# adamjorr/kbbq

Hardware: AMD Instinct MI355X
Metric: recalibrated Gbases/sec (higher is better)
Workload: dtype u64

## Files before the change

### kbbq_amd/csrc/bucket.h

```cpp
#pragma once
#include <hip/hip_runtime.h>
#include <stdint.h>

#include "device_common.h"

namespace kbbq {

constexpr int SUB_BITS = 12;
constexpr int NB2_BITS = 9;
constexpr int SUB_BLOCKS = 1 << SUB_BITS;
constexpr int NB2 = 1 << NB2_BITS;
constexpr int L1_SHIFT = SUB_BITS + NB2_BITS;
constexpr int MAX_NB1 = 512;
constexpr int N_XCD = 8;
constexpr int CNT_STRIDE = 32;
constexpr int BK_THREADS = 512;
constexpr int EMIT_GRID = 512;

struct BucketDev {
    unsigned long long *l1;
    uint32_t *l1_cnt;
    uint32_t *l2;
    uint32_t *l2_cnt;
    uint32_t *tickets;
    unsigned long long *direct;
    uint32_t cap1, cap2;
    int nb1;
    int n_src;
    int cnt_stride;
    uint32_t n_sub;
};

__device__ __forceinline__ int xcc_id() {
    unsigned x;
    asm volatile("s_getreg_b32 %0, hwreg(HW_REG_XCC_ID, 0, 4)" : "=s"(x));
    return (int)(x & (N_XCD - 1));
}

__device__ __forceinline__ uint32_t block_scan512(uint32_t v, uint32_t *wave_tot, uint32_t *total) {
    const int lane = threadIdx.x & 63, w = threadIdx.x >> 6;
    uint32_t inc = v;
#pragma unroll
    for (int o = 1; o < 64; o <<= 1) { const uint32_t y = __shfl_up(inc, o); if (lane >= o) inc += y; }
    if (lane == 63) wave_tot[w] = inc;
    __syncthreads();
    uint32_t before = 0, all = 0;
#pragma unroll
    for (int i = 0; i < 8; ++i) { const uint32_t t = wave_tot[i]; before += i < w ? t : 0; all += t; }
    *total = all;
    return before + inc - v;
}

template <int NW, int CH, bool BY_BASE, int RPW, bool PRIV, bool DENSE = true>
__global__ void __launch_bounds__(BK_THREADS) k_emit_marked(ReadsDev R, KParams K, FiltDev F, BucketDev B, const uint64_t *mask,
                                                             uint64_t mask_words, const uint64_t *kofs,
                                                             unsigned long long *inserted) {
    using S = Stage<NW>;
    constexpr int SLOTS = RPW * CH;
    extern __shared__ unsigned long long sorted[];
    __shared__ uint32_t stage[8][DENSE ? RPW : 1][2 * S::WORDS];
    __shared__ uint32_t hist[MAX_NB1], ofs_l[MAX_NB1], gbase_l[MAX_NB1], fill_l[MAX_NB1], wave_tot[8];
    const int lane = threadIdx.x & 63;
    const int w = __builtin_amdgcn_readfirstlane(threadIdx.x >> 6);
    uint32_t *L32 = stage[w][0];
    const int k = K.k;
    const int src = PRIV ? (int)blockIdx.x : xcc_id();
    const uint64_t reads_per_tile = 8 * RPW;
    const uint64_t n_tiles = (R.n_reads + reads_per_tile - 1) / reads_per_tile;
    unsigned long long mine = 0, direct = 0;
    hist[threadIdx.x] = 0;
    if (PRIV) fill_l[threadIdx.x] = (int)threadIdx.x < B.nb1 ? B.l1_cnt[(size_t)src * B.nb1 + threadIdx.x] : 0u;
    __syncthreads();
    uint64_t off[RPW], kb[RPW], word[RPW];
    uint32_t len[RPW];
    auto fetch_tile = [&](uint64_t tile) {
        const uint64_t r0 = (tile * 8 + w) * RPW;
#pragma unroll
        for (int rr = 0; rr < RPW; ++rr) {
            off[rr] = 0; kb[rr] = 0; word[rr] = 0; len[rr] = 0;
            if (r0 + rr < R.n_reads) {
                read_span(R, r0 + rr, off[rr], len[rr]);
                kb[rr] = BY_BASE ? off[rr] : kmer_base(kofs, r0 + rr, R.read_len, k);
                word[rr] = stage_fetch<NW>(R, nullptr, mask, kb[rr], mask_words - 1, off[rr], lane);
            }
        }
    };
    if (blockIdx.x < n_tiles) fetch_tile(blockIdx.x);
    for (uint64_t tile = blockIdx.x; tile < n_tiles; tile += gridDim.x) {
        unsigned long long rec[SLOTS];
        int rk[SLOTS];
#pragma unroll
        for (int s = 0; s < SLOTS; ++s) { rec[s] = 0; rk[s] = -1; }
        if (DENSE) {
            unsigned long long *wlist = sorted + (size_t)w * SLOTS * 64;
            int n_dense = 0;
            __builtin_amdgcn_wave_barrier();
            if (lane < S::WORDS) {
#pragma unroll
                for (int rr = 0; rr < RPW; ++rr) stage_store(stage[w][rr], lane, word[rr]);
            }
            __builtin_amdgcn_wave_barrier();
#pragma unroll
            for (int rr = 0; rr < RPW; ++rr) {
                const int nk = (int)len[rr] - k + 1;
                if (nk > 0) {
                    const uint32_t *L32 = stage[w][rr];
                    const int o31 = (int)(off[rr] & 31), o63 = (int)(off[rr] & 63), x63 = (int)(kb[rr] & 63);
#pragma unroll
                    for (int c = 0; c < CH; ++c) {
                        if (c * 64 < nk) {
                            const int s = c * 64 + lane;
                            const bool marked = lds_bit(L32 + 2 * S::X, x63 + s) != 0;
                            const bool valid = (lds_window32(L32 + 2 * S::M, o63 + s) & K.nmask_bits) == 0;
                            const bool take = s < nk && marked && (BY_BASE || valid);
                            const unsigned long long bal = __ballot(take);
                            if (take) wlist[n_dense + __popcll(bal & ((1ULL << lane) - 1))] = lds_window64(L32 + 2 * S::B, 2 * (o31 + s));
                            n_dense += (int)__popcll(bal);
                            if (!BY_BASE && R.hint_sampled) or_bits64(R.hint_sampled, off[rr] + (uint64_t)c * 64, bal, lane);
                            mine += __popcll(bal);
                        }
                    }
                }
            }
            __builtin_amdgcn_wave_barrier();
#pragma unroll
            for (int i = 0; i < SLOTS; ++i) {
                if (i * 64 < n_dense && i * 64 + lane < n_dense) {
                    const uint64_t key = canon_key(wlist[i * 64 + lane], K);
                    const uint32_t blk = block_of(F, key);
                    rec[i] = ((unsigned long long)blk << 16) | pattern_of(F, key);
                    rk[i] = (int)atomicAdd(&hist[blk >> L1_SHIFT], 1u);
                }
            }
        } else {
#pragma unroll
        for (int rr = 0; rr < RPW; ++rr) {
            const int nk = (int)len[rr] - k + 1;
            if (nk > 0) {
                __builtin_amdgcn_wave_barrier();
                if (lane < S::WORDS) stage_store(L32, lane, word[rr]);
                __builtin_amdgcn_wave_barrier();
                const int o31 = (int)(off[rr] & 31), o63 = (int)(off[rr] & 63), x63 = (int)(kb[rr] & 63);
#pragma unroll
                for (int c = 0; c < CH; ++c) {
                    if (c * 64 < nk) {
                        const int s = c * 64 + lane;
                        const bool marked = lds_bit(L32 + 2 * S::X, x63 + s) != 0;
                        const bool valid = (lds_window32(L32 + 2 * S::M, o63 + s) & K.nmask_bits) == 0;
                        const bool take = s < nk && marked && (BY_BASE || valid);
                        const uint64_t key = canon_key(lds_window64(L32 + 2 * S::B, 2 * (o31 + s)), K);
                        const uint32_t blk = block_of(F, key);
                        rec[rr * CH + c] = ((unsigned long long)blk << 16) | pattern_of(F, key);
                        if (take) rk[rr * CH + c] = (int)atomicAdd(&hist[blk >> L1_SHIFT], 1u);
                        const unsigned long long bal = __ballot(take);
                        if (!BY_BASE && R.hint_sampled) or_bits64(R.hint_sampled, off[rr] + (uint64_t)c * 64, bal, lane);
                        mine += __popcll(bal);
                    }
                }
            }
        }
        }
        if (tile + gridDim.x < n_tiles) fetch_tile(tile + gridDim.x);
        __syncthreads();
        const uint32_t cnt = hist[threadIdx.x];
        hist[threadIdx.x] = 0;
        uint32_t g = 0;
        if (PRIV) {
            g = fill_l[threadIdx.x];
            fill_l[threadIdx.x] = g + cnt;
        } else if (cnt) {
            g = atomicAdd(&B.l1_cnt[((size_t)src * B.nb1 + threadIdx.x) * CNT_STRIDE], cnt);
        }
        uint32_t total;
        const uint32_t ex = block_scan512(cnt, wave_tot, &total);
        ofs_l[threadIdx.x] = ex;
        gbase_l[threadIdx.x] = g;
        __syncthreads();
#pragma unroll
        for (int s = 0; s < SLOTS; ++s)
            if (rk[s] >= 0) sorted[ofs_l[(uint32_t)(rec[s] >> (16 + L1_SHIFT))] + (uint32_t)rk[s]] = rec[s];
        __syncthreads();
        for (uint32_t i = threadIdx.x; i < total; i += BK_THREADS) {
            const unsigned long long v = sorted[i];
            const uint32_t b = (uint32_t)(v >> (16 + L1_SHIFT));
            const uint32_t pos = gbase_l[b] + (i - ofs_l[b]);
            if (pos < B.cap1) {
                B.l1[((size_t)src * B.nb1 + b) * B.cap1 + pos] = v;
            } else {
                bloom_put(F, (uint32_t)(v >> 16), (uint32_t)(v & 0xFFFFu));
                ++direct;
            }
        }
        if (DENSE) __syncthreads();
    }
    if (PRIV && (int)threadIdx.x < B.nb1) B.l1_cnt[(size_t)src * B.nb1 + threadIdx.x] = fill_l[threadIdx.x];
    if (inserted && lane == 0 && mine) atomicAdd(inserted, mine);
    if (direct) atomicAdd(B.direct, direct);
}

constexpr int SPLIT_PER_THREAD = 12;
constexpr int SPLIT_TILE = BK_THREADS * SPLIT_PER_THREAD;

__global__ void __launch_bounds__(BK_THREADS) k_split(FiltDev F, BucketDev B, uint32_t chunks_per_region) {
    __shared__ uint32_t hist[NB2], ofs_l[NB2], gbase_l[NB2], wave_tot[8], unit_l;
    __shared__ uint32_t sorted[SPLIT_TILE];
    __shared__ uint16_t sorted_b[SPLIT_TILE];
    const int home = xcc_id();
    unsigned long long direct = 0;
    hist[threadIdx.x] = 0;
    for (int qi = 0; qi < N_XCD; ++qi) {
        const int q = (home + qi) & (N_XCD - 1);
        const uint32_t n_buckets = B.nb1 > q ? (uint32_t)(B.nb1 - q + N_XCD - 1) / N_XCD : 0;
        const uint32_t n_units = n_buckets * (uint32_t)B.n_src * chunks_per_region;
        for (;;) {
            __syncthreads();
            if (threadIdx.x == 0) unit_l = atomicAdd(&B.tickets[q * CNT_STRIDE], 1u);
            __syncthreads();
            const uint32_t unit = unit_l;
            if (unit >= n_units) break;
            const uint32_t chunk = unit % chunks_per_region, rest = unit / chunks_per_region;
            const int x = (int)(rest % (uint32_t)B.n_src), b1 = q + (int)(rest / (uint32_t)B.n_src) * N_XCD;
            const size_t region = (size_t)x * B.nb1 + b1;
            const uint32_t n = min(B.l1_cnt[region * B.cnt_stride], B.cap1);
            const uint32_t first = chunk * (uint32_t)SPLIT_TILE;
            if (first >= n) continue;
            const uint32_t m = min((uint32_t)SPLIT_TILE, n - first);
            const unsigned long long *src = B.l1 + region * B.cap1 + first;
            uint32_t rec[SPLIT_PER_THREAD];
            int rk[SPLIT_PER_THREAD];
#pragma unroll
            for (int j = 0; j < SPLIT_PER_THREAD; ++j) {
                const uint32_t i = j * BK_THREADS + threadIdx.x;
// ... 92 lines not shown
```

### kbbq_amd/csrc/engine.hip

```cpp
#include <hip/hip_runtime.h>

#include <algorithm>
#include <cstdarg>
#include <cstdio>
#include <cstdlib>
#include <cstring>
#include <map>
#include <mutex>
#include <string>
#include <thread>
#include <vector>

#include "../../include/kbbq_engine.h"
#include "abi_internal.h"
#include "correct.h"
#include "correct_wave.h"
#include "device_common.h"
#include "host_model.h"

using namespace kbbq;

static thread_local char g_err[512] = "";
int kbbq_fail(int code, const char *fmt, ...) {
    va_list ap;
// ... 24 lines not shown
    uint64_t table_bytes() const { return spec.n_blocks * kEngineBlockBytes; }
    FiltDev dev() const {
        FiltDev f;
        f.table = reinterpret_cast<ulonglong2 *>(d_table);
        f.patterns = reinterpret_cast<const ulonglong2 *>(d_patterns);
        f.n_blocks = spec.n_blocks;
        const ModMagic mm = make_mod_magic(spec.n_blocks);
        f.mod_magic = mm.m64;
        f.mod_m32 = mm.m32;
        f.salt0 = spec.salt[0];
        f.salt1 = spec.salt[1];
        return f;
    }
};

struct ProfileSlot {
    std::string name;
    uint64_t launches = 0;
    double ms = 0;
};
struct PendingEvent {
    int slot;
    hipEvent_t a, b;
};

struct Options {
    bool no_overlap = false;
    bool no_fastpath = false;
    bool lane_walk = false;
    bool no_pass4_pipeline = false;
    int pass2_side = 2;
    bool tally_general = false;
    bool infer_subset = true;
    bool debug_bucket = false;
    int bucket = -1;
    uint64_t bucket_records = 0;
    uint64_t pass4_piece = 0;
    int scan_blocks = -1;
    int walk_blocks = -1;
    int infer_blocks = 0;
};

struct kbbq_engine {
    kbbq_params p;
    Options opt;
    KParams K;
    hipStream_t stream = nullptr;
    hipStream_t stream2 = nullptr;
    hipEvent_t ev_main = nullptr, ev_side[2] = {nullptr, nullptr};
    hipEvent_t ev_draw = nullptr, ev_ins[2] = {nullptr, nullptr};
    bool ins_pending[2] = {false, false};
    int draw_turn = 0;
    bool side_busy[2] = {false, false};
    bool pass3_shared = false;
    unsigned long long *d_totals = nullptr;
    int side_turn = 0;
    uint32_t *d_qpresent = nullptr;
    uint32_t qpresent[8] = {};
    bool qpresent_known = false;
    uint8_t *d_dq_qslot = nullptr;
    int dq_slots = 0;
    uint32_t *d_rg_present[2] = {nullptr, nullptr};
    hipStream_t cur = nullptr;
    unsigned long long *cur_cnt = nullptr;
    FilterHost filt[2];
    Xoshiro256 seed_state;
    uint64_t draw_threshold = 0;
    bool draw_always = false;
    bool thresholds_set = false;
    std::vector<int32_t> thresholds;
    unsigned long long *d_hist = nullptr;
    uint64_t hist_cycle_words = 0, hist_dinuc_words = 0;
    DqTables dq;
// ... 552 lines not shown

int kbbq_engine_create(const kbbq_params *params, kbbq_engine **out) {
    if (!params || !out) return fail(KBBQ_EINVAL, "null argument");
    if (params->k < 1 || params->k > KBBQ_MAX_KMER) return fail(KBBQ_ERANGE, "k must be <= %d and > 0", KBBQ_MAX_KMER);
    if (params->n_rg < 1 || params->n_rg > 65535) return fail(KBBQ_EINVAL, "n_rg must be in 1..65535");
    if (params->max_read_len < 1 || params->max_read_len > KBBQ_MAX_READ_LEN)
        return fail(KBBQ_ERANGE, "max_read_len must be in 1..%d", KBBQ_MAX_READ_LEN);
    int ndev = 0;
    if (hipGetDeviceCount(&ndev) != hipSuccess || ndev == 0) return fail(KBBQ_ENODEV, "no HIP device visible");
    if (params->device < 0 || params->device >= ndev) return fail(KBBQ_ENODEV, "device %d of %d", params->device, ndev);
    DeviceGuard create_guard(params->device);
    HIP_TRY(create_guard.err);
    kbbq_engine *e = new kbbq_engine;
    e->p = *params;
    {
        Options &o = e->opt;
        auto env_set = [](const char *name) { const char *v = getenv(name); return v && *v; };
        auto env_int = [](const char *name, int dflt) { const char *v = getenv(name); return v && *v ? atoi(v) : dflt; };
        const int fl = params->flags;
        o.no_overlap = (fl & KBBQ_F_NO_OVERLAP) || env_set("KBBQ_NO_OVERLAP");
        o.no_fastpath = (fl & KBBQ_F_NO_FASTPATH) || env_set("KBBQ_NO_FASTPATH");
        o.lane_walk = (fl & KBBQ_F_LANE_WALK) || (getenv("KBBQ_CORRECT") && !strcmp(getenv("KBBQ_CORRECT"), "lane"));
        o.no_pass4_pipeline = (fl & KBBQ_F_NO_PASS4_PIPELINE) || env_set("KBBQ_NO_PASS4_PIPELINE");
        o.pass2_side = (fl & KBBQ_F_PASS2_INORDER) ? 0 : env_int("KBBQ_PASS2_SIDE", o.pass2_side);
        o.tally_general = env_set("KBBQ_TALLY_GENERAL");
        o.infer_subset = env_int("KBBQ_INFER_SUBSET", 1) != 0;
        o.debug_bucket = env_set("KBBQ_DEBUG_BUCKET");
        o.bucket = (fl & KBBQ_F_BUCKET_ON) ? 1 : (fl & KBBQ_F_BUCKET_OFF) ? 0 : env_set("KBBQ_BUCKET") ? (env_int("KBBQ_BUCKET", 0) != 0 ? 1 : 0) : -1;
        o.bucket_records = env_u64("KBBQ_BUCKET_RECORDS", 0);
        o.pass4_piece = env_u64("KBBQ_PASS4_PIECE", 0);
        o.scan_blocks = env_int("KBBQ_SCAN_BLOCKS", o.scan_blocks);
        o.walk_blocks = env_int("KBBQ_WALK_BLOCKS", o.walk_blocks);
        o.infer_blocks = env_int("KBBQ_INFER_BLOCKS", o.infer_blocks);
    }
    e->K.k = params->k;
    e->K.shift = 2u * (unsigned)(params->k - 1);
    e->K.mask = params->k < 32 ? ((1ULL << (2 * params->k)) - 1) : ~0ULL;
    e->K.nmask_bits = params->k < 32 ? ((1u << params->k) - 1) : 0xFFFFFFFFu;
    const double fprs[2] = {params->fpr_sampled, params->fpr_trusted};
    for (int w = 0; w < 2; ++w) {
        if (!make_filter_spec(params->approx_kmers, fprs[w], params->bloom_seed, e->filt[w].spec)) {
            delete e;
            return fail(KBBQ_EINVAL, "Error: Invalid bloom filter parameters. Adjust parameters and try again.");
        }
    }
    hipError_t he = hipStreamCreateWithFlags(&e->stream, hipStreamNonBlocking);
    if (he == hipSuccess) he = hipStreamCreateWithFlags(&e->stream2, hipStreamNonBlocking);
    if (he == hipSuccess) he = hipEventCreateWithFlags(&e->ev_main, hipEventDisableTiming);
    if (he == hipSuccess) he = hipEventCreateWithFlags(&e->ev_draw, hipEventDisableTiming);
    for (int t = 0; t < 2 && he == hipSuccess; ++t) he = hipEventCreateWithFlags(&e->ev_ins[t], hipEventDisableTiming);
    if (he == hipSuccess) he = hipEventCreateWithFlags(&e->ev_side[0], hipEventDisableTiming);
    if (he == hipSuccess) he = hipEventCreateWithFlags(&e->ev_side[1], hipEventDisableTiming);
    if (he == hipSuccess) he = hipStreamCreateWithFlags(&e->copy, hipStreamNonBlocking);
    if (he == hipSuccess) he = hipEventCreateWithFlags(&e->bk.ev_flush, hipEventDisableTiming);
    if (he == hipSuccess) he = hipEventCreateWithFlags(&e->bk.ev_est, hipEventDisableTiming);
    if (he == hipSuccess) he = hipEventCreateWithFlags(&e->ev_infer, hipEventDisableTiming);
    for (int t = 0; t < 2 && he == hipSuccess; ++t) he = hipEventCreateWithFlags(&e->ev_take[t], hipEventDisableTiming);
    if (he == hipSuccess) he = hipHostMalloc((void **)&e->bk.h_inserted, 64, hipHostMallocDefault);
    for (int i = 0; i < 3 && he == hipSuccess; ++i) {
        he = hipEventCreateWithFlags(&e->slot[i].h2d, hipEventDisableTiming);
        if (he == hipSuccess) he = hipEventCreateWithFlags(&e->slot[i].d2h, hipEventDisableTiming);
        for (int t = 0; t < 2 && he == hipSuccess; ++t) he = hipEventCreateWithFlags(&e->slot[i].done[t], hipEventDisableTiming);
    }
    e->cur = e->stream;
    if (he != hipSuccess) { kbbq_engine_destroy(e); return fail(KBBQ_EIO, "hipStreamCreate: %s", hipGetErrorString(he)); }
#define CREATE_TRY(expr)                                                                           \
// ... 123 lines not shown
    e->dq_set = false;
    memset(e->stats, 0, sizeof e->stats);
    return sync_engine(e);
}

int kbbq_engine_sync(kbbq_engine *e) {
    ENGINE_DEVICE(e);
    { int frc = bucket_flush_all(e); if (frc) return frc; }
    if (!e) return fail(KBBQ_EINVAL, "null engine");
    return sync_engine(e);
}

void *kbbq_engine_stream(kbbq_engine *e) { return e ? (void *)e->stream : nullptr; }

int kbbq_engine_dims(kbbq_engine *e, uint64_t *n_rg, uint64_t *n_cycle) {
    if (!e) return fail(KBBQ_EINVAL, "null engine");
    if (n_rg) *n_rg = (uint64_t)e->p.n_rg;
    if (n_cycle) *n_cycle = (uint64_t)e->p.max_read_len;
    return KBBQ_OK;
}

int kbbq_engine_tune(kbbq_engine *e, const char *name, uint64_t value) {
    if (!e || !name) return fail(KBBQ_EINVAL, "null argument");
    if (!strcmp(name, "bucket_records")) {
        if (e->bk.allocated) return fail(KBBQ_ESTATE, "the record buffers are allocated already");
        e->opt.bucket_records = value;
    } else if (!strcmp(name, "pass4_piece")) {
        e->opt.pass4_piece = value;
    } else if (!strcmp(name, "scan_blocks") || !strcmp(name, "walk_blocks") || !strcmp(name, "infer_blocks")) {
        if (value > 17) return fail(KBBQ_EINVAL, "%s: 0 (as many as fit) to 16 workgroups per CU, 17 = default", name);
        (name[0] == 's' ? e->opt.scan_blocks : name[0] == 'w' ? e->opt.walk_blocks : e->opt.infer_blocks) = value == 17 ? (name[0] == 'i' ? 0 : -1) : (int)value;
    } else if (!strcmp(name, "infer_subset")) {
        e->opt.infer_subset = value != 0;
    } else if (!strcmp(name, "pass2_side")) {
        ENGINE_DEVICE(e);
        { int frc = bucket_flush_all(e); if (frc) return frc; }
        int rc = sync_engine(e);
        if (rc) return rc;
        if (value > 2) return fail(KBBQ_EINVAL, "pass2_side: 0, 1 or 2");
        e->opt.pass2_side = (int)value;
        e->bk.stream[0] = e->bk.stream[1] = nullptr;
    } else if (!strcmp(name, "no_overlap")) {
        ENGINE_DEVICE(e);
        { int frc = bucket_flush_all(e); if (frc) return frc; }
        int rc = sync_engine(e);
        if (rc) return rc;
        e->opt.no_overlap = value != 0;
        e->bk.stream[0] = e->bk.stream[1] = nullptr;
    } else {
        return fail(KBBQ_EINVAL, "unknown knob '%s'", name);
    }
    return KBBQ_OK;
}

int kbbq_filter_info_get(kbbq_engine *e, int which, kbbq_filter_info *out) {
    ENGINE_DEVICE(e);
    { int frc = bucket_flush_all(e); if (frc) return frc; }
    if (!e || !out || which < 0 || which > 1) return fail(KBBQ_EINVAL, "bad argument");
    const FilterSpec &s = e->filt[which].spec;
    memset(out, 0, sizeof *out);
    out->bits = s.bits;
    out->bits_unblocked = s.bits_unblocked;
    out->n_blocks = s.n_blocks;
    out->table_bytes = e->filt[which].table_bytes();
    out->random_seed = s.random_seed;
    out->n_hash = s.n_hash;
// ... 459 lines not shown

int kbbq_count_kmer_positions(kbbq_engine *e, const kbbq_reads *reads, uint64_t *out) {
    ENGINE_DEVICE(e);
    if (!e || !reads || !out) return fail(KBBQ_EINVAL, "null argument");
    HostBatchDone host_done(e, reads);
    ReadsDev R; int max_len;
    int rc = device_view(e, reads, &R, &max_len, false);
    if (rc) return rc;
    const uint64_t *kofs;
    return kmer_prefix(e, R, &kofs, out);
}

}

constexpr int kStagedMax = 512;
constexpr int kTallyMaxWindows = 24;
template <template <int> class Launcher, typename... Args>
static int dispatch_nw(int max_len, Args... args) {
    if (max_len <= 192) return Launcher<3>::go(args...);
    if (max_len <= 320) return Launcher<5>::go(args...);
    return Launcher<8>::go(args...);
}

template <int NW> struct LaunchSample {
    static int go(kbbq_engine *e, ReadsDev R, const uint64_t *mask, uint64_t mask_words, const uint64_t *kofs) {
        Timed t(e, "k_insert_sampled");
        hipLaunchKernelGGL((k_insert_marked<NW, false>), dim3(wave_grid(R.n_reads)), dim3(256), 0, e->stream, R, e->K,
                           e->filt[0].dev(), mask, mask_words, kofs, e->filt[0].d_inserted);
        HIP_TRY(hipGetLastError());
        return KBBQ_OK;
    }
};

template <int NW, int CH, int RPW>
static int launch_emit(kbbq_engine *e, int w, ReadsDev R, const uint64_t *mask, uint64_t mask_words, const uint64_t *kofs,
                       unsigned long long *inserted) {
    const BucketDev B = bucket_dev(e, w);
    const uint64_t n_tiles = (R.n_reads + 8 * RPW - 1) / (8 * RPW);
    const int grid = (int)std::min<uint64_t>(n_tiles, EMIT_GRID);
    const size_t lds = (size_t)8 * RPW * CH * 64 * 8;
    hipStream_t st = bucket_stream(e, w);
    Timed t(e, w ? "k_emit_trusted" : "k_emit_sampled", st);
#define KBBQ_EMIT(BYB)                                                                                                        \
    do {                                                                                                                      \
        const void *fn = (const void *)k_emit_marked<NW, CH, BYB, RPW, true, true>;                                            \
        size_t &raised = e->attr_lds_correct[fn];                                                                             \
        if (lds > 48 * 1024 && lds > raised) {                                                                                \
            HIP_TRY(hipFuncSetAttribute(fn, hipFuncAttributeMaxDynamicSharedMemorySize, (int)lds));                            \
            raised = lds;                                                                                                     \
        }                                                                                                                     \
        hipLaunchKernelGGL((k_emit_marked<NW, CH, BYB, RPW, true, true>), dim3(grid), dim3(BK_THREADS), lds, st, R, e->K,      \
                           e->filt[w].dev(), B, mask, mask_words, kofs, inserted);                                            \
    } while (0)
    if (w == 0) KBBQ_EMIT(false); else KBBQ_EMIT(true);
#undef KBBQ_EMIT
    HIP_TRY(hipGetLastError());
    return KBBQ_OK;
}

static int dispatch_emit(kbbq_engine *e, int w, int max_len, ReadsDev R, const uint64_t *mask, uint64_t mask_words, const uint64_t *kofs,
                         unsigned long long *inserted) {
    const int max_nk = std::max(1, max_len - e->p.k + 1);
    if (max_len <= 192) {
        if (max_nk <= 128) return launch_emit<3, 2, 4>(e, w, R, mask, mask_words, kofs, inserted);
        return launch_emit<3, 3, 4>(e, w, R, mask, mask_words, kofs, inserted);
    }
    if (max_len <= 320) return launch_emit<5, 5, 2>(e, w, R, mask, mask_words, kofs, inserted);
    return launch_emit<8, 8, 1>(e, w, R, mask, mask_words, kofs, inserted);
}

extern "C" {

int kbbq_sample_batch(kbbq_engine *e, const kbbq_reads *reads, uint64_t first_kmer_ordinal) {
    ENGINE_DEVICE(e);
    if (!e) return fail(KBBQ_EINVAL, "null engine");
    HostBatchDone host_done(e, reads);
    ReadsDev R; int max_len;
    int rc = device_view(e, reads, &R, &max_len, false);
    if (rc) return rc;
    const uint64_t *kofs; uint64_t n_draws;
    if ((rc = kmer_prefix(e, R, &kofs, &n_draws))) return rc;
    if (n_draws == 0) return KBBQ_OK;
    const bool overlap = reads->on_device && !e->opt.no_overlap;
    const int turn = overlap ? e->draw_turn : 0;
    const int slot = turn ? 13 : 0;
    if ((rc = ensure_scratch(e, slot, (n_draws / 64 + 2) * 8))) return rc;
    uint64_t *mask = (uint64_t *)e->scratch[slot];
    hipStream_t ds = overlap ? e->stream2 : e->stream;
    if (overlap) {
        e->draw_turn ^= 1;
        if (e->ins_pending[turn]) HIP_TRY(hipStreamWaitEvent(ds, e->ev_ins[turn], 0));
    }
    {
        Timed t(e, "k_draw_mask", ds);
        const uint64_t lanes = (n_draws + DRAWS_PER_LANE - 1) / DRAWS_PER_LANE;
        uint64_t st[4];
        xoshiro_state_at(e->p.seed, first_kmer_ordinal, st);
        hipLaunchKernelGGL(k_draw_mask, dim3((unsigned)((lanes + 255) / 256)), dim3(256), 0, ds,
                           st[0], st[1], st[2], st[3],
                           (uint64_t)0, n_draws, e->draw_threshold, e->draw_always ? 1 : 0, mask);
        HIP_TRY(hipGetLastError());
    }
    if (overlap) {
        HIP_TRY(hipEventRecord(e->ev_draw, ds));
        HIP_TRY(hipStreamWaitEvent(e->stream, e->ev_draw, 0));
    }
    if (max_len > kStagedMax) {
        Timed t(e, "k_insert_sampled_long");
        hipLaunchKernelGGL(k_insert_marked_long<false>, dim3(wave_grid(R.n_reads)), dim3(256), 0, e->stream, R, e->K, e->filt[0].dev(),
                           (const uint64_t *)mask, n_draws / 64 + 2, kofs, e->filt[0].d_inserted);
        HIP_TRY(hipGetLastError());
        rc = KBBQ_OK;
    } else if (bucket_on(e, 0)) {
        if ((rc = bucket_reserve(e, 0, (double)n_draws * std::min(1.0, e->p.alpha) * 1.01 + 4096.0, R.n_bases))) return rc;
        rc = dispatch_emit(e, 0, max_len, R, (const uint64_t *)mask, n_draws / 64 + 2, kofs, e->filt[0].d_inserted);
    } else {
        rc = dispatch_nw<LaunchSample>(max_len, e, R, (const uint64_t *)mask, n_draws / 64 + 2, kofs);
    }
    if (!rc) {
        HIP_TRY(hipEventRecord(e->ev_ins[turn], e->stream));
        e->ins_pending[turn] = true;
    }
    return rc;
}

int kbbq_sample_finish(kbbq_engine *e, uint64_t *inserted) {
    ENGINE_DEVICE(e);
    { int frc = bucket_flush_all(e); if (frc) return frc; }
    if (!e) return fail(KBBQ_EINVAL, "null engine");
    int rc = sync_engine(e);
    if (rc) return rc;
    if (inserted) HIP_TRY(hipMemcpy(inserted, e->filt[0].d_inserted, 8, hipMemcpyDeviceToHost));
    return KBBQ_OK;
}

int kbbq_compute_thresholds(kbbq_engine *e, const char *alpha_text, int32_t *thresholds_out, double *fpr_out,
                            char *p_text_out, size_t p_text_len) {
    ENGINE_DEVICE(e);
    { int frc = bucket_flush_all(e); if (frc) return frc; }
    if (!e || !alpha_text) return fail(KBBQ_EINVAL, "null argument");
    int rc = sync_engine(e);
    if (rc) return rc;
    uint64_t inserted = 0;
    HIP_TRY(hipMemcpy(&inserted, e->filt[0].d_inserted, 8, hipMemcpyDeviceToHost));
    if (inserted == 0) return fail(KBBQ_ESTATE, "no k-mers were sampled");
    double fpr = 0;
    std::string p_text;
    e->thresholds = thresholds_from_counts(e->p.k, e->filt[0].spec.bits, inserted, e->filt[0].spec.n_salt, alpha_text, &fpr, &p_text);
// ... 34 lines not shown
template <int NW> struct LaunchTrusted {
    static int go(kbbq_engine *e, ReadsDev R, uint32_t *take_bits, uint32_t *err_out, int max_len) {
        Thresholds thr;
        memset(&thr, 0, sizeof thr);
        for (size_t i = 0; i < e->thresholds.size() && i <= KBBQ_MAX_KMER; ++i) thr.v[i] = e->thresholds[i];
        HIP_TRY(hipMemsetAsync(e->d_tickets, 0, 4, e->stream));
        {
            Timed t(e, "k_infer");
            int edge = -1, pmask = 3;
            if (e->opt.infer_subset && !infer_subset_plan(e->thresholds, e->p.k, &edge, &pmask)) edge = -1;
            if (edge >= 0 && getenv("KBBQ_SUBSET_EDGE")) edge = atoi(getenv("KBBQ_SUBSET_EDGE"));
            if (edge >= 0 && getenv("KBBQ_SUBSET_PMASK")) pmask = atoi(getenv("KBBQ_SUBSET_PMASK"));
            const bool short_nk = std::max(1, max_len - e->p.k + 1) <= (NW - 1) * 64;
#define KBBQ_LAUNCH_INFER(NK_, SUB_)                                                                                              \
    hipLaunchKernelGGL((k_infer<NW, NK_, 1, SUB_>), dim3(wave_grid(R.n_reads, shared_cap(e, e->opt.infer_blocks))), dim3(256), 0, e->stream, R, e->K, e->filt[0].dev(), thr, \
                       take_bits, e->filt[1].d_inserted, err_out, e->d_qpresent, e->d_counters + 3, e->d_tickets, edge, pmask)
            if (edge >= 0) { if (short_nk) KBBQ_LAUNCH_INFER(NW - 1, true); else KBBQ_LAUNCH_INFER(NW, true); }
            else { if (short_nk) KBBQ_LAUNCH_INFER(NW - 1, false); else KBBQ_LAUNCH_INFER(NW, false); }
#undef KBBQ_LAUNCH_INFER
            HIP_TRY(hipGetLastError());
        }
        if (bucket_on(e, 1)) {
            const bool side = e->opt.pass2_side != 0 && !e->opt.no_overlap;
            e->bk.stream[1] = side ? e->stream2 : e->stream;
            if (side) {
                HIP_TRY(hipEventRecord(e->ev_infer, e->stream));
                HIP_TRY(hipStreamWaitEvent(e->stream2, e->ev_infer, 0));
                e->cur_slot_side = true;
            }
            bucket_poll_estimate(e);
            e->bk.frac_used = e->bk.frac_trusted;
            int rc = bucket_reserve(e, 1, (double)R.n_bases * e->bk.frac_trusted + 4096.0, R.n_bases);
            if (rc) return rc;
            return dispatch_emit(e, 1, max_len, R, (const uint64_t *)take_bits, R.n_bases / 64 + 2, (const uint64_t *)nullptr,
                                 (unsigned long long *)nullptr);
        }
        {
            Timed t(e, "k_insert_trusted");
            hipLaunchKernelGGL((k_insert_marked<NW, true>), dim3(wave_grid(R.n_reads)), dim3(256), 0, e->stream, R, e->K,
                               e->filt[1].dev(), (const uint64_t *)take_bits, R.n_bases / 64 + 2,
                               (const uint64_t *)nullptr, (unsigned long long *)nullptr);
            HIP_TRY(hipGetLastError());
        }
        return KBBQ_OK;
    }
};
extern "C" {

static int bit_out_begin(kbbq_engine *e, const kbbq_reads *reads, uint64_t *user, int slot, uint32_t **dev) {
    *dev = nullptr;
    if (!user) return KBBQ_OK;
    const size_t bytes = (reads->n_bases / 64 + 2) * 8;
    if (reads->on_device) {
        *dev = (uint32_t *)user;
    } else {
        int rc = ensure_scratch(e, slot, bytes);
        if (rc) return rc;
        *dev = (uint32_t *)e->scratch[slot];
    }
    HIP_TRY(hipMemsetAsync(*dev, 0, (reads->n_bases / 64 + 1) * 8, e->stream));
    return KBBQ_OK;
}
static int bit_out_end(kbbq_engine *e, const kbbq_reads *reads, uint64_t *user, uint32_t *dev) {
    if (!user || reads->on_device) return KBBQ_OK;
    HIP_TRY(hipMemcpyAsync(user, dev, (reads->n_bases / 64 + 1) * 8, hipMemcpyDeviceToHost, e->stream));
    HIP_TRY(hipStreamSynchronize(e->stream));
    return KBBQ_OK;
// ... 762 lines not shown
```

Baseline: 23.08.

## Add append-style emit kernel with register-ballot take masks as default

Adds a new emit kernel that computes the per-k-mer take mask from the fetched words in registers using readlane and funnel shifts, instead of reading bits from LDS. It appends records directly into each bucket through LDS atomic fill counters, replacing the per-tile histogram, block scan and LDS sort. It also moves the next-tile prefetch earlier and drops the per-tile __syncthreads. The old sort-per-tile kernel stays available behind a new emit_form knob, with its non-dense and non-private branches removed. The trade-off is scattered global writes into buckets, where the old kernel wrote them grouped after a sort.

After: 21.74. 5.8% lower.

```diff
diff --git a/kbbq_amd/csrc/bucket.h b/kbbq_amd/csrc/bucket.h
--- a/kbbq_amd/csrc/bucket.h
+++ b/kbbq_amd/csrc/bucket.h
@@ -51,25 +51,131 @@
     return before + inc - v;
 }
 
-template <int NW, int CH, bool BY_BASE, int RPW, bool PRIV, bool DENSE = true>
+
+__device__ __forceinline__ uint64_t wave_word(uint64_t v, int src_lane) {
+    const uint32_t lo = (uint32_t)__builtin_amdgcn_readlane((int)(uint32_t)v, src_lane);
+    const uint32_t hi = (uint32_t)__builtin_amdgcn_readlane((int)(uint32_t)(v >> 32), src_lane);
+    return ((uint64_t)hi << 32) | lo;
+}
+__device__ __forceinline__ uint64_t funnel64(uint64_t lo, uint64_t hi, int sh) { return (lo >> sh) | ((hi << 1) << (63 - sh)); }
+
+template <int NW, bool BY_BASE>
+__device__ __forceinline__ uint64_t emit_take(uint64_t word, int c, int nk, int o63, int x63, uint32_t nmask_bits, int lane) {
+    using S = Stage<NW>;
+    const int left = nk - c * 64;
+    uint64_t take = funnel64(wave_word(word, S::X + c), wave_word(word, S::X + c + 1), x63);
+    take &= left >= 64 ? ~0ULL : (1ULL << left) - 1;
+    if (!BY_BASE) {
+        const uint64_t m0 = wave_word(word, S::M + c), m1 = wave_word(word, S::M + c + 1), m2 = wave_word(word, S::M + c + 2);
+        const uint64_t a = funnel64(m0, m1, o63), b = funnel64(m1, m2, o63);
+        take &= __ballot(((uint32_t)funnel64(a, b, lane) & nmask_bits) == 0);
+    }
+    return take;
+}
+
+template <int NW, int CH, bool BY_BASE, int RPW>
+__global__ void __launch_bounds__(BK_THREADS) k_emit_append(ReadsDev R, KParams K, FiltDev F, BucketDev B, const uint64_t *mask,
+                                                             uint64_t mask_words, const uint64_t *kofs,
+                                                             unsigned long long *inserted) {
+    using S = Stage<NW>;
+    constexpr int SLOTS = RPW * CH;
+    extern __shared__ unsigned long long wlists[];
+    __shared__ uint32_t stage[8][RPW][2 * S::NB];
+    __shared__ uint32_t fill_l[MAX_NB1];
+    __shared__ unsigned long long base_l[MAX_NB1];
+    const int lane = threadIdx.x & 63;
+    const int w = __builtin_amdgcn_readfirstlane(threadIdx.x >> 6);
+    const int k = K.k;
+    const size_t src = blockIdx.x;
+    const uint64_t reads_per_tile = 8 * RPW;
+    const uint64_t n_tiles = (R.n_reads + reads_per_tile - 1) / reads_per_tile;
+    const uint32_t cap1 = B.cap1;
+    unsigned long long mine = 0, direct = 0;
+    fill_l[threadIdx.x] = (int)threadIdx.x < B.nb1 ? B.l1_cnt[src * B.nb1 + threadIdx.x] : 0u;
+    base_l[threadIdx.x] = (unsigned long long)(src * B.nb1 + threadIdx.x) * cap1;
+    __syncthreads();
+    unsigned long long *wlist = wlists + (size_t)w * SLOTS * 64;
+    uint64_t off[RPW], kb[RPW], word[RPW];
+    uint32_t len[RPW];
+    auto fetch_tile = [&](uint64_t tile) {
+        const uint64_t r0 = (tile * 8 + w) * RPW;
+#pragma unroll
+        for (int rr = 0; rr < RPW; ++rr) {
+            off[rr] = 0; kb[rr] = 0; word[rr] = 0; len[rr] = 0;
+            if (r0 + rr < R.n_reads) {
+                read_span(R, r0 + rr, off[rr], len[rr]);
+                kb[rr] = BY_BASE ? off[rr] : kmer_base(kofs, r0 + rr, R.read_len, k);
+                word[rr] = stage_fetch<NW>(R, nullptr, mask, kb[rr], mask_words - 1, off[rr], lane);
+            }
+        }
+    };
+    if (blockIdx.x < n_tiles) fetch_tile(blockIdx.x);
+    for (uint64_t tile = blockIdx.x; tile < n_tiles; tile += gridDim.x) {
+        int n_dense = 0;
+        __builtin_amdgcn_wave_barrier();
+        if (lane < S::NB) {
+#pragma unroll
+            for (int rr = 0; rr < RPW; ++rr) stage_store(stage[w][rr], lane, word[rr]);
+        }
+        __builtin_amdgcn_wave_barrier();
+#pragma unroll
+        for (int rr = 0; rr < RPW; ++rr) {
+            const int nk = (int)len[rr] - k + 1;
+            const int o31 = (int)(off[rr] & 31), o63 = (int)(off[rr] & 63), x63 = (int)(kb[rr] & 63);
+#pragma unroll
+            for (int c = 0; c < CH; ++c) {
+                if (c * 64 < nk) {
+                    const uint64_t take = emit_take<NW, BY_BASE>(word[rr], c, nk, o63, x63, K.nmask_bits, lane);
+                    if ((take >> lane) & 1)
+                        wlist[n_dense + __popcll(take & ((1ULL << lane) - 1))] = lds_window64(stage[w][rr], 2 * (o31 + c * 64 + lane));
+                    n_dense += (int)__popcll(take);
+                    if (!BY_BASE && R.hint_sampled) or_bits64(R.hint_sampled, off[rr] + (uint64_t)c * 64, take, lane);
+                }
+            }
+        }
+        mine += n_dense;
+        __builtin_amdgcn_wave_barrier();
+        if (tile + gridDim.x < n_tiles) fetch_tile(tile + gridDim.x);
+#pragma unroll
+        for (int i = 0; i < SLOTS; ++i) {
+            if (i * 64 < n_dense && i * 64 + lane < n_dense) {
+                const uint64_t key = canon_key(wlist[i * 64 + lane], K);
+                const uint32_t blk = block_of(F, key), pat = pattern_of(F, key);
+                const uint32_t b = blk >> L1_SHIFT;
+                const uint32_t pos = atomicAdd(&fill_l[b], 1u);
+                if (pos < cap1) {
+                    B.l1[base_l[b] + pos] = ((unsigned long long)blk << 16) | pat;
+                } else {
+                    bloom_put(F, blk, pat);
+                    ++direct;
+                }
+            }
+        }
+    }
+    __syncthreads();
+    if ((int)threadIdx.x < B.nb1) B.l1_cnt[src * B.nb1 + threadIdx.x] = fill_l[threadIdx.x];
+    if (inserted && lane == 0 && mine) atomicAdd(inserted, mine);
+    if (direct) atomicAdd(B.direct, direct);
+}
+
+template <int NW, int CH, bool BY_BASE, int RPW>
 __global__ void __launch_bounds__(BK_THREADS) k_emit_marked(ReadsDev R, KParams K, FiltDev F, BucketDev B, const uint64_t *mask,
                                                              uint64_t mask_words, const uint64_t *kofs,
                                                              unsigned long long *inserted) {
     using S = Stage<NW>;
     constexpr int SLOTS = RPW * CH;
     extern __shared__ unsigned long long sorted[];
-    __shared__ uint32_t stage[8][DENSE ? RPW : 1][2 * S::WORDS];
+    __shared__ uint32_t stage[8][RPW][2 * S::WORDS];
     __shared__ uint32_t hist[MAX_NB1], ofs_l[MAX_NB1], gbase_l[MAX_NB1], fill_l[MAX_NB1], wave_tot[8];
     const int lane = threadIdx.x & 63;
     const int w = __builtin_amdgcn_readfirstlane(threadIdx.x >> 6);
-    uint32_t *L32 = stage[w][0];
     const int k = K.k;
-    const int src = PRIV ? (int)blockIdx.x : xcc_id();
+    const int src = (int)blockIdx.x;
     const uint64_t reads_per_tile = 8 * RPW;
     const uint64_t n_tiles = (R.n_reads + reads_per_tile - 1) / reads_per_tile;
     unsigned long long mine = 0, direct = 0;
     hist[threadIdx.x] = 0;
-    if (PRIV) fill_l[threadIdx.x] = (int)threadIdx.x < B.nb1 ? B.l1_cnt[(size_t)src * B.nb1 + threadIdx.x] : 0u;
+    fill_l[threadIdx.x] = (int)threadIdx.x < B.nb1 ? B.l1_cnt[(size_t)src * B.nb1 + threadIdx.x] : 0u;
     __syncthreads();
     uint64_t off[RPW], kb[RPW], word[RPW];
     uint32_t len[RPW];
@@ -91,55 +197,19 @@
         int rk[SLOTS];
 #pragma unroll
         for (int s = 0; s < SLOTS; ++s) { rec[s] = 0; rk[s] = -1; }
-        if (DENSE) {
-            unsigned long long *wlist = sorted + (size_t)w * SLOTS * 64;
-            int n_dense = 0;
-            __builtin_amdgcn_wave_barrier();
-            if (lane < S::WORDS) {
-#pragma unroll
-                for (int rr = 0; rr < RPW; ++rr) stage_store(stage[w][rr], lane, word[rr]);
-            }
-            __builtin_amdgcn_wave_barrier();
-#pragma unroll
-            for (int rr = 0; rr < RPW; ++rr) {
-                const int nk = (int)len[rr] - k + 1;
-                if (nk > 0) {
-                    const uint32_t *L32 = stage[w][rr];
-                    const int o31 = (int)(off[rr] & 31), o63 = (int)(off[rr] & 63), x63 = (int)(kb[rr] & 63);
-#pragma unroll
-                    for (int c = 0; c < CH; ++c) {
-                        if (c * 64 < nk) {
-                            const int s = c * 64 + lane;
-                            const bool marked = lds_bit(L32 + 2 * S::X, x63 + s) != 0;
-                            const bool valid = (lds_window32(L32 + 2 * S::M, o63 + s) & K.nmask_bits) == 0;
-                            const bool take = s < nk && marked && (BY_BASE || valid);
-                            const unsigned long long bal = __ballot(take);
-                            if (take) wlist[n_dense + __popcll(bal & ((1ULL << lane) - 1))] = lds_window64(L32 + 2 * S::B, 2 * (o31 + s));
-                            n_dense += (int)__popcll(bal);
-                            if (!BY_BASE && R.hint_sampled) or_bits64(R.hint_sampled, off[rr] + (uint64_t)c * 64, bal, lane);
-                            mine += __popcll(bal);
-                        }
-                    }
-                }
-            }
-            __builtin_amdgcn_wave_barrier();
-#pragma unroll
-            for (int i = 0; i < SLOTS; ++i) {
-                if (i * 64 < n_dense && i * 64 + lane < n_dense) {
-                    const uint64_t key = canon_key(wlist[i * 64 + lane], K);
-                    const uint32_t blk = block_of(F, key);
-                    rec[i] = ((unsigned long long)blk << 16) | pattern_of(F, key);
-                    rk[i] = (int)atomicAdd(&hist[blk >> L1_SHIFT], 1u);
-                }
-            }
-        } else {
+        unsigned long long *wlist = sorted + (size_t)w * SLOTS * 64;
+        int n_dense = 0;
+        __builtin_amdgcn_wave_barrier();
+        if (lane < S::WORDS) {
+#pragma unroll
+            for (int rr = 0; rr < RPW; ++rr) stage_store(stage[w][rr], lane, word[rr]);
+        }
+        __builtin_amdgcn_wave_barrier();
 #pragma unroll
         for (int rr = 0; rr < RPW; ++rr) {
             const int nk = (int)len[rr] - k + 1;
             if (nk > 0) {
-                __builtin_amdgcn_wave_barrier();
-                if (lane < S::WORDS) stage_store(L32, lane, word[rr]);
-                __builtin_amdgcn_wave_barrier();
+                const uint32_t *L32 = stage[w][rr];
                 const int o31 = (int)(off[rr] & 31), o63 = (int)(off[rr] & 63), x63 = (int)(kb[rr] & 63);
 #pragma unroll
                 for (int c = 0; c < CH; ++c) {
@@ -148,29 +218,31 @@
                         const bool marked = lds_bit(L32 + 2 * S::X, x63 + s) != 0;
                         const bool valid = (lds_window32(L32 + 2 * S::M, o63 + s) & K.nmask_bits) == 0;
                         const bool take = s < nk && marked && (BY_BASE || valid);
-                        const uint64_t key = canon_key(lds_window64(L32 + 2 * S::B, 2 * (o31 + s)), K);
-                        const uint32_t blk = block_of(F, key);
-                        rec[rr * CH + c] = ((unsigned long long)blk << 16) | pattern_of(F, key);
-                        if (take) rk[rr * CH + c] = (int)atomicAdd(&hist[blk >> L1_SHIFT], 1u);
                         const unsigned long long bal = __ballot(take);
+                        if (take) wlist[n_dense + __popcll(bal & ((1ULL << lane) - 1))] = lds_window64(L32 + 2 * S::B, 2 * (o31 + s));
+                        n_dense += (int)__popcll(bal);
                         if (!BY_BASE && R.hint_sampled) or_bits64(R.hint_sampled, off[rr] + (uint64_t)c * 64, bal, lane);
                         mine += __popcll(bal);
                     }
                 }
             }
         }
+        __builtin_amdgcn_wave_barrier();
+#pragma unroll
+        for (int i = 0; i < SLOTS; ++i) {
+            if (i * 64 < n_dense && i * 64 + lane < n_dense) {
+                const uint64_t key = canon_key(wlist[i * 64 + lane], K);
+                const uint32_t blk = block_of(F, key);
+                rec[i] = ((unsigned long long)blk << 16) | pattern_of(F, key);
+                rk[i] = (int)atomicAdd(&hist[blk >> L1_SHIFT], 1u);
+            }
         }
         if (tile + gridDim.x < n_tiles) fetch_tile(tile + gridDim.x);
         __syncthreads();
         const uint32_t cnt = hist[threadIdx.x];
         hist[threadIdx.x] = 0;
-        uint32_t g = 0;
-        if (PRIV) {
-            g = fill_l[threadIdx.x];
-            fill_l[threadIdx.x] = g + cnt;
-        } else if (cnt) {
-            g = atomicAdd(&B.l1_cnt[((size_t)src * B.nb1 + threadIdx.x) * CNT_STRIDE], cnt);
-        }
+        const uint32_t g = fill_l[threadIdx.x];
+        fill_l[threadIdx.x] = g + cnt;
         uint32_t total;
         const uint32_t ex = block_scan512(cnt, wave_tot, &total);
         ofs_l[threadIdx.x] = ex;
@@ -191,9 +263,9 @@
                 ++direct;
             }
         }
-        if (DENSE) __syncthreads();
-    }
-    if (PRIV && (int)threadIdx.x < B.nb1) B.l1_cnt[(size_t)src * B.nb1 + threadIdx.x] = fill_l[threadIdx.x];
+        __syncthreads();
+    }
+    if ((int)threadIdx.x < B.nb1) B.l1_cnt[(size_t)src * B.nb1 + threadIdx.x] = fill_l[threadIdx.x];
     if (inserted && lane == 0 && mine) atomicAdd(inserted, mine);
     if (direct) atomicAdd(B.direct, direct);
 }
diff --git a/kbbq_amd/csrc/engine.hip b/kbbq_amd/csrc/engine.hip
--- a/kbbq_amd/csrc/engine.hip
+++ b/kbbq_amd/csrc/engine.hip
@@ -80,6 +80,7 @@
     int pass2_side = 2;
     bool tally_general = false;
     bool infer_subset = true;
+    int emit_form = 0;
     bool debug_bucket = false;
     int bucket = -1;
     uint64_t bucket_records = 0;
@@ -894,6 +895,9 @@
         (name[0] == 's' ? e->opt.scan_blocks : name[0] == 'w' ? e->opt.walk_blocks : e->opt.infer_blocks) = value == 17 ? (name[0] == 'i' ? 0 : -1) : (int)value;
     } else if (!strcmp(name, "infer_subset")) {
         e->opt.infer_subset = value != 0;
+    } else if (!strcmp(name, "emit_form")) {
+        if (value > 1) return fail(KBBQ_EINVAL, "emit_form: 0 (append) or 1 (sort per tile)");
+        e->opt.emit_form = (int)value;
     } else if (!strcmp(name, "pass2_side")) {
         ENGINE_DEVICE(e);
         { int frc = bucket_flush_all(e); if (frc) return frc; }
@@ -1428,18 +1432,22 @@
     const size_t lds = (size_t)8 * RPW * CH * 64 * 8;
     hipStream_t st = bucket_stream(e, w);
     Timed t(e, w ? "k_emit_trusted" : "k_emit_sampled", st);
-#define KBBQ_EMIT(BYB)                                                                                                        \
+#define KBBQ_EMIT(KERNEL, BYB)                                                                                                \
     do {                                                                                                                      \
-        const void *fn = (const void *)k_emit_marked<NW, CH, BYB, RPW, true, true>;                                            \
+        const void *fn = (const void *)KERNEL<NW, CH, BYB, RPW>;                                                              \
         size_t &raised = e->attr_lds_correct[fn];                                                                             \
         if (lds > 48 * 1024 && lds > raised) {                                                                                \
             HIP_TRY(hipFuncSetAttribute(fn, hipFuncAttributeMaxDynamicSharedMemorySize, (int)lds));                            \
             raised = lds;                                                                                                     \
         }                                                                                                                     \
-        hipLaunchKernelGGL((k_emit_marked<NW, CH, BYB, RPW, true, true>), dim3(grid), dim3(BK_THREADS), lds, st, R, e->K,      \
-                           e->filt[w].dev(), B, mask, mask_words, kofs, inserted);                                            \
+        hipLaunchKernelGGL((KERNEL<NW, CH, BYB, RPW>), dim3(grid), dim3(BK_THREADS), lds, st, R, e->K, e->filt[w].dev(), B,    \
+                           mask, mask_words, kofs, inserted);                                                                 \
     } while (0)
-    if (w == 0) KBBQ_EMIT(false); else KBBQ_EMIT(true);
+    if (e->opt.emit_form == 0) {
+        if (w == 0) KBBQ_EMIT(k_emit_append, false); else KBBQ_EMIT(k_emit_append, true);
+    } else {
+        if (w == 0) KBBQ_EMIT(k_emit_marked, false); else KBBQ_EMIT(k_emit_marked, true);
+    }
 #undef KBBQ_EMIT
     HIP_TRY(hipGetLastError());
     return KBBQ_OK;
```

## Add mark-driven bucket emit kernel that compacts set mask bits before hashing

Applied to the files above, without the earlier changes.

Adds a new emit kernel that scans the sample/trusted bit mask per tile, compacts set bits into an LDS list, and only loads bases and hashes k-mers at marked positions, then bins records by L1 bucket as before. It replaces walking every read and every k-mer in the emit path for fixed-length reads, for both the sampled and trusted passes by default. The intent is to avoid work on unmarked positions when marks are sparse. In exchange it uses large dynamic LDS, which limits occupancy, and does per-mark random base loads.

Measured after the change: 23.67 before, 24.72 after, median of 4. 1.04x the previous value.

```diff
diff --git a/kbbq_amd/csrc/bucket.h b/kbbq_amd/csrc/bucket.h
--- a/kbbq_amd/csrc/bucket.h
+++ b/kbbq_amd/csrc/bucket.h
@@ -198,6 +198,147 @@
     if (direct) atomicAdd(B.direct, direct);
 }
 
+constexpr int MARK_TILE = 8 * BK_THREADS;
+constexpr int MARK_LIST = 32 * BK_THREADS;
+constexpr int MARK_SLOTS = 4;
+constexpr size_t MARK_LDS = (size_t)MARK_TILE * 8 + (size_t)MARK_LIST * 2;
+
+struct MarkPlan {
+    uint64_t n_bits;
+    uint64_t n_tiles;
+    uint32_t tile_bits;
+    uint32_t div;
+    uint32_t inv;
+    uint32_t nk;
+    uint32_t tile_reads;
+    uint32_t pieces;
+    uint32_t x_bits;
+    uint32_t tiles_per_round;
+};
+
+__device__ __forceinline__ void or_bits_ascending(uint32_t *bits, uint64_t pos, bool set, int lane) {
+    const uint32_t wd = (uint32_t)(pos >> 5);
+    uint32_t v = set ? 1u << (pos & 31) : 0u;
+#pragma unroll
+    for (int o = 1; o < 32; o <<= 1) {
+        const uint32_t y = __shfl_down(v, o), wy = __shfl_down(wd, o);
+        if (wy == wd) v |= y;
+    }
+    const uint32_t wp = __shfl_up(wd, 1);
+    if ((lane == 0 || wp != wd) && v) atomicOr(&bits[wd], v);
+}
+
+template <bool BY_BASE>
+__global__ void __launch_bounds__(BK_THREADS) k_emit_by_mark(ReadsDev R, KParams K, FiltDev F, BucketDev B, const uint32_t *mask,
+                                                              MarkPlan P, unsigned long long *inserted) {
+    extern __shared__ unsigned long long sorted[];
+    uint16_t *list = reinterpret_cast<uint16_t *>(sorted + MARK_TILE);
+    __shared__ uint32_t hist[MAX_NB1], ofs_l[MAX_NB1], gbase_l[MAX_NB1], fill_l[MAX_NB1], wave_tot[8], list_tot[8];
+    const int lane = threadIdx.x & 63;
+    const uint32_t w64 = (uint32_t)__builtin_amdgcn_readfirstlane(threadIdx.x >> 6) * 64u;
+    const int src = (int)blockIdx.x;
+    const uint32_t *bases32 = reinterpret_cast<const uint32_t *>(R.bases);
+    const uint32_t *nmask32 = reinterpret_cast<const uint32_t *>(R.nmask);
+    const uint32_t q = threadIdx.x / P.pieces, pi = threadIdx.x - q * P.pieces;
+    const uint64_t my_tiles = blockIdx.x < P.n_tiles ? (P.n_tiles - blockIdx.x + gridDim.x - 1) / gridDim.x : 0;
+    const uint64_t n_rounds = (my_tiles + P.tiles_per_round - 1) / P.tiles_per_round;
+    const uint32_t x_mask = (1u << P.x_bits) - 1u;
+    unsigned long long mine = 0, direct = 0;
+    hist[threadIdx.x] = 0;
+    fill_l[threadIdx.x] = (int)threadIdx.x < B.nb1 ? B.l1_cnt[(size_t)src * B.nb1 + threadIdx.x] : 0u;
+    __syncthreads();
+    auto fetch_piece = [&](uint64_t round) -> uint32_t {
+        const uint64_t mt = round * P.tiles_per_round + q;
+        if (q >= P.tiles_per_round || mt >= my_tiles) return 0u;
+        const uint64_t lo = (blockIdx.x + mt * gridDim.x) * P.tile_bits, hi = min(lo + P.tile_bits, P.n_bits);
+        const uint64_t pw = (lo >> 5) + pi, pb = pw << 5;
+        if (pb >= hi) return 0u;
+        uint32_t v = mask[pw];
+        if (pb < lo) v &= ~0u << (uint32_t)(lo - pb);
+        if (hi - pb < 32) v &= (1u << (uint32_t)(hi - pb)) - 1u;
+        return v;
+    };
+    uint32_t next = fetch_piece(0);
+    for (uint64_t round = 0; round < n_rounds; ++round) {
+        const uint32_t piece = next;
+        if (round + 1 < n_rounds) next = fetch_piece(round + 1);
+        uint32_t n_list;
+        uint32_t at = block_scan512((uint32_t)__popc(piece), list_tot, &n_list);
+        for (uint32_t v = piece; v; v &= v - 1) list[at++] = (uint16_t)((q << P.x_bits) | (pi * 32u + (uint32_t)(__ffs((int)v) - 1)));
+        __syncthreads();
+        const uint32_t round_tile0 = (uint32_t)(blockIdx.x + round * P.tiles_per_round * gridDim.x);
+        for (uint32_t t0 = 0; t0 < n_list; t0 += MARK_TILE) {
+            unsigned long long rec[8];
+            int rk[8];
+#pragma unroll
+            for (int s = 0; s < 8; ++s) { rec[s] = 0; rk[s] = -1; }
+#pragma unroll
+            for (int h = 0; h < 8; h += MARK_SLOTS) {
+                uint32_t a0[MARK_SLOTS], a1[MARK_SLOTS], a2[MARK_SLOTS], m0[MARK_SLOTS], m1[MARK_SLOTS];
+                uint64_t b[MARK_SLOTS];
+                bool ok[MARK_SLOTS];
+#pragma unroll
+                for (int s = 0; s < MARK_SLOTS; ++s) {
+                    const uint32_t j = t0 + (uint32_t)(h + s) * BK_THREADS + w64 + lane;
+                    const uint32_t e = list[min(j, n_list - 1)];
+                    const uint32_t tile = round_tile0 + (e >> P.x_bits) * gridDim.x;
+                    const uint32_t y = (e & x_mask) - ((tile * P.tile_bits) & 31u);
+                    const uint32_t r = P.div == 1 ? y : __umulhi(y, P.inv), start = y - r * P.div;
+                    b[s] = (uint64_t)(tile * P.tile_reads + r) * R.read_len + start;
+                    ok[s] = j < n_list && start < P.nk;
+                    const uint32_t *pb = bases32 + (b[s] >> 4);
+                    a0[s] = pb[0]; a1[s] = pb[1]; a2[s] = pb[2];
+                    m0[s] = m1[s] = 0;
+                    if (!BY_BASE) { const uint32_t *pn = nmask32 + (b[s] >> 5); m0[s] = pn[0]; m1[s] = pn[1]; }
+                }
+#pragma unroll
+                for (int s = 0; s < MARK_SLOTS; ++s) {
+                    if (t0 + (uint32_t)(h + s) * BK_THREADS + w64 < n_list) {
+                        const int sh = 2 * (int)(b[s] & 15);
+                        const uint64_t win = (uint64_t)__builtin_amdgcn_alignbit(a1[s], a0[s], sh) | ((uint64_t)__builtin_amdgcn_alignbit(a2[s], a1[s], sh) << 32);
+                        const bool valid = BY_BASE || (__builtin_amdgcn_alignbit(m1[s], m0[s], (int)(b[s] & 31)) & K.nmask_bits) == 0;
+                        const bool take = ok[s] && valid;
+                        const uint64_t key = canon_key(win, K);
+                        const uint32_t blk = block_of(F, key);
+                        rec[h + s] = ((unsigned long long)blk << 16) | pattern_of(F, key);
+                        if (take) rk[h + s] = (int)atomicAdd(&hist[blk >> L1_SHIFT], 1u);
+                        mine += __popcll(__ballot(take));
+                        if (!BY_BASE && R.hint_sampled) or_bits_ascending(R.hint_sampled, b[s], take, lane);
+                    }
+                }
+            }
+            __syncthreads();
+            const uint32_t cnt = hist[threadIdx.x];
+            hist[threadIdx.x] = 0;
+            const uint32_t g = fill_l[threadIdx.x];
+            fill_l[threadIdx.x] = g + cnt;
+            uint32_t total;
+            const uint32_t ex = block_scan512(cnt, wave_tot, &total);
+            ofs_l[threadIdx.x] = ex;
+            gbase_l[threadIdx.x] = g;
+            __syncthreads();
+#pragma unroll
+            for (int s = 0; s < 8; ++s)
+                if (rk[s] >= 0) sorted[ofs_l[(uint32_t)(rec[s] >> (16 + L1_SHIFT))] + (uint32_t)rk[s]] = rec[s];
+            __syncthreads();
+            for (uint32_t i = threadIdx.x; i < total; i += BK_THREADS) {
+                const unsigned long long v = sorted[i];
+                const uint32_t bk = (uint32_t)(v >> (16 + L1_SHIFT));
+                const uint32_t pos = gbase_l[bk] + (i - ofs_l[bk]);
+                if (pos < B.cap1) {
+                    B.l1[((size_t)src * B.nb1 + bk) * B.cap1 + pos] = v;
+                } else {
+                    bloom_put(F, (uint32_t)(v >> 16), (uint32_t)(v & 0xFFFFu));
+                    ++direct;
+                }
+            }
+        }
+    }
+    if ((int)threadIdx.x < B.nb1) B.l1_cnt[(size_t)src * B.nb1 + threadIdx.x] = fill_l[threadIdx.x];
+    if (inserted && lane == 0 && mine) atomicAdd(inserted, mine);
+    if (direct) atomicAdd(B.direct, direct);
+}
+
 constexpr int SPLIT_PER_THREAD = 12;
 constexpr int SPLIT_TILE = BK_THREADS * SPLIT_PER_THREAD;
 
diff --git a/kbbq_amd/csrc/engine.hip b/kbbq_amd/csrc/engine.hip
--- a/kbbq_amd/csrc/engine.hip
+++ b/kbbq_amd/csrc/engine.hip
@@ -87,6 +87,7 @@
     int scan_blocks = -1;
     int walk_blocks = -1;
     int infer_blocks = 0;
+    int emit_by_read = 0;
 };
 
 struct kbbq_engine {
@@ -705,6 +706,7 @@
         o.scan_blocks = env_int("KBBQ_SCAN_BLOCKS", o.scan_blocks);
         o.walk_blocks = env_int("KBBQ_WALK_BLOCKS", o.walk_blocks);
         o.infer_blocks = env_int("KBBQ_INFER_BLOCKS", o.infer_blocks);
+        o.emit_by_read = std::min(2, std::max(0, env_int("KBBQ_EMIT_BY_READ", o.emit_by_read)));
     }
     e->K.k = params->k;
     e->K.shift = 2u * (unsigned)(params->k - 1);
@@ -894,6 +896,9 @@
         (name[0] == 's' ? e->opt.scan_blocks : name[0] == 'w' ? e->opt.walk_blocks : e->opt.infer_blocks) = value == 17 ? (name[0] == 'i' ? 0 : -1) : (int)value;
     } else if (!strcmp(name, "infer_subset")) {
         e->opt.infer_subset = value != 0;
+    } else if (!strcmp(name, "emit_by_read")) {
+        if (value > 2) return fail(KBBQ_EINVAL, "emit_by_read: 0 (the engine's choice), 1 (by read) or 2 (by mark in pass 2 too)");
+        e->opt.emit_by_read = (int)value;
     } else if (!strcmp(name, "pass2_side")) {
         ENGINE_DEVICE(e);
         { int frc = bucket_flush_all(e); if (frc) return frc; }
@@ -1419,6 +1424,8 @@
     }
 };
 
+constexpr bool kPass2ByMark = true;
+
 template <int NW, int CH, int RPW>
 static int launch_emit(kbbq_engine *e, int w, ReadsDev R, const uint64_t *mask, uint64_t mask_words, const uint64_t *kofs,
                        unsigned long long *inserted) {
@@ -1445,9 +1452,43 @@
     return KBBQ_OK;
 }
 
-static int dispatch_emit(kbbq_engine *e, int w, int max_len, ReadsDev R, const uint64_t *mask, uint64_t mask_words, const uint64_t *kofs,
-                         unsigned long long *inserted) {
+static int launch_emit_by_mark(kbbq_engine *e, int w, uint32_t tile_reads, ReadsDev R, const uint64_t *mask, uint64_t n_marks,
+                               unsigned long long *inserted) {
+    const BucketDev B = bucket_dev(e, w);
+    MarkPlan P;
+    P.n_bits = n_marks;
+    P.n_tiles = (R.n_reads + tile_reads - 1) / tile_reads;
+    P.nk = R.read_len - (uint32_t)e->p.k + 1;
+    P.div = w ? R.read_len : P.nk;
+    P.inv = (uint32_t)(((1ULL << 32) + P.div - 1) / P.div);
+    P.tile_reads = tile_reads;
+    P.tile_bits = tile_reads * P.div;
+    P.pieces = (P.tile_bits + 62) / 32;
+    P.x_bits = 5;
+    while ((1u << P.x_bits) < P.pieces * 32) ++P.x_bits;
+    P.tiles_per_round = std::min<uint32_t>(BK_THREADS / P.pieces, 1u << (16 - P.x_bits));
+    const int grid = (int)std::min<uint64_t>(P.n_tiles, EMIT_GRID);
+    hipStream_t st = bucket_stream(e, w);
+    Timed t(e, w ? "k_emit_trusted" : "k_emit_sampled", st);
+    const void *fn = w ? (const void *)k_emit_by_mark<true> : (const void *)k_emit_by_mark<false>;
+    size_t &raised = e->attr_lds_correct[fn];
+    if (MARK_LDS > raised) {
+        HIP_TRY(hipFuncSetAttribute(fn, hipFuncAttributeMaxDynamicSharedMemorySize, (int)MARK_LDS));
+        raised = MARK_LDS;
+    }
+    if (w) hipLaunchKernelGGL(k_emit_by_mark<true>, dim3(grid), dim3(BK_THREADS), MARK_LDS, st, R, e->K, e->filt[w].dev(), B, (const uint32_t *)mask, P, inserted);
+    else hipLaunchKernelGGL(k_emit_by_mark<false>, dim3(grid), dim3(BK_THREADS), MARK_LDS, st, R, e->K, e->filt[w].dev(), B, (const uint32_t *)mask, P, inserted);
+    HIP_TRY(hipGetLastError());
+    return KBBQ_OK;
+}
+
+static int dispatch_emit(kbbq_engine *e, int w, int max_len, ReadsDev R, const uint64_t *mask, uint64_t mask_words, uint64_t n_marks,
+                         const uint64_t *kofs, unsigned long long *inserted) {
     const int max_nk = std::max(1, max_len - e->p.k + 1);
+    const uint32_t tile_reads = max_len <= 192 ? 32 : max_len <= 320 ? 16 : 8;
+    const bool by_mark = e->opt.emit_by_read != 1 && (w == 0 || e->opt.emit_by_read == 2 || kPass2ByMark) && !R.offsets &&
+                         R.read_len >= (uint32_t)e->p.k && R.read_len <= (uint32_t)kStagedMax && R.n_reads < (1ULL << 32) && R.n_bases < (1ULL << 36);
+    if (by_mark) return launch_emit_by_mark(e, w, tile_reads, R, mask, n_marks, inserted);
     if (max_len <= 192) {
         if (max_nk <= 128) return launch_emit<3, 2, 4>(e, w, R, mask, mask_words, kofs, inserted);
         return launch_emit<3, 3, 4>(e, w, R, mask, mask_words, kofs, inserted);
@@ -1500,7 +1541,7 @@
         rc = KBBQ_OK;
     } else if (bucket_on(e, 0)) {
         if ((rc = bucket_reserve(e, 0, (double)n_draws * std::min(1.0, e->p.alpha) * 1.01 + 4096.0, R.n_bases))) return rc;
-        rc = dispatch_emit(e, 0, max_len, R, (const uint64_t *)mask, n_draws / 64 + 2, kofs, e->filt[0].d_inserted);
+        rc = dispatch_emit(e, 0, max_len, R, (const uint64_t *)mask, n_draws / 64 + 2, n_draws, kofs, e->filt[0].d_inserted);
     } else {
         rc = dispatch_nw<LaunchSample>(max_len, e, R, (const uint64_t *)mask, n_draws / 64 + 2, kofs);
     }
@@ -1601,7 +1642,7 @@
             e->bk.frac_used = e->bk.frac_trusted;
             int rc = bucket_reserve(e, 1, (double)R.n_bases * e->bk.frac_trusted + 4096.0, R.n_bases);
             if (rc) return rc;
-            return dispatch_emit(e, 1, max_len, R, (const uint64_t *)take_bits, R.n_bases / 64 + 2, (const uint64_t *)nullptr,
+            return dispatch_emit(e, 1, max_len, R, (const uint64_t *)take_bits, R.n_bases / 64 + 2, R.n_bases, (const uint64_t *)nullptr,
                                  (unsigned long long *)nullptr);
         }
         {
```
